# normallytangent/dune-eigensolver

Measured on AMD Instinct MI355X. Metric: Lanczos iters/sec + achieved SpMV HBM GB/s, 3D Poisson 256^3, higher is better.
Workload: dtype f64

## Files before the change

### dune-eigensolver_amd/csrc/drivers.cpp

```cpp
#include <algorithm>
#include <complex>
#include <cmath>
#include <cstdlib>
#include <cstring>
#include <numeric>
#include <string>
#include <vector>

#include "internal.h"

using namespace eigmi;

namespace {

bool distributed(const eig_mat_s &A) { return A.ctx->distributed(); }

struct PinnedDoubles {
  double *p = nullptr, *dev = nullptr;
  explicit PinnedDoubles(size_t n)
  {
    EIG_HIP(hipHostMalloc(reinterpret_cast<void **>(&p), (n ? n : 1) * sizeof(double), hipHostMallocMapped));
    EIG_HIP(hipHostGetDevicePointer(reinterpret_cast<void **>(&dev), p, 0));
  }
  ~PinnedDoubles()
// ... 1113 lines not shown
    EIG_CHECK(mode == EIG_ARNOLDI_STD || mode == EIG_ARNOLDI_GEN, EIG_ERR_ARG, "eig_arnoldi_shift_invert: bad mode");
    shift_invert_check(A, B);
    EIG_HIP(hipSetDevice(A->ctx->device));
    LuRef F;
    shift_invert_factor(A, B, lu, sigma, F);
    arnoldi_core(A, B, F, sigma, nev, ncv, tol, maxit, seed, mode == EIG_ARNOLDI_GEN, eval_re, eval_im, evec_host,
                 restarts);
  });
}

namespace {

struct LanczosBufs {
  DevBuf scal;
  DevBuf ictl;
  LanczosState st;
  double *carry;
  explicit LanczosBufs(int steps, int launches = 0)
      : scal((size_t)(4 * (steps + 2) + 6 * (launches + 2) + 8) * sizeof(double)),
        ictl((size_t)2 * (launches + 2) * sizeof(int))
  {
    double *b = scal.d();
    st.dsum = b;
    st.nsum = b + (steps + 2);
    st.alpha = b + 2 * (steps + 2);
    st.beta = b + 3 * (steps + 2);
    st.fred = b + 4 * (steps + 2);
    st.aux = st.fred + 3 * (launches + 2);
    carry = st.aux + 2 * (launches + 2);
    st.mu2 = carry + 4;
    st.pn = st.mu2 + 4;
    st.ctl = static_cast<int *>(ictl.p);
  }
};

enum { kPartOnly = 0, kPartFirst = 1, kPartSecond = 2 };
template <class Halo, class Launch>
void halo_split(eig_mat_s &A, hipEvent_t e0, hipEvent_t e1, Halo halo, Launch launch)
{
  eig_ctx_t ctx = A.ctx;
  hipStream_t s = ctx->stream;
  if (!distributed(A) || (A.recvs.empty() && A.sends.empty()))
  {
    launch(nullptr, 0, A.nslices, kPartOnly);
    return;
  }
  if (ctx->loop)
// ... 56 lines not shown
                        int nev, hipEvent_t halo_ev0, hipEvent_t halo_ev1, bool ev_external, int xch = 0)
{
  eig_ctx_t ctx = A.ctx;
  hipStream_t s = ctx->stream;
  auto mark = [&](int i) {
    if (ev && i < nev)
      EIG_HIP(hipEventRecordWithFlags(ev[i], s, ev_external ? hipEventRecordExternal : hipEventRecordDefault));
  };
  double *out = lb.st.fred + 3 * (i64)L;
  FusedLaunch fl{lb.st, L, force, xch & kXchPublish};
  FusedLaunch fl_first{lb.st, L, force, 0};
  mark(0);
  halo_split(
      A, halo_ev0, halo_ev1, [&](hipStream_t hs) { halo_exchange(A, P, hs, nullptr, 2); },
      [&](const i32 *sl, i64 first, i64 count, int part) {
        launch_lanczos_fused(A, P, Pout, part == kPartFirst ? fl_first : fl, sl, first, count,
                             part == kPartSecond ? lb.carry : nullptr, part == kPartFirst ? lb.carry : out, 0, s,
                             ctx->red);
      });
  mark(1);
  if (!(xch & kXchPublish)) allreduce_sum(ctx, out, 3, s);
  mark(2);
  mark(3);
  mark(4);
}

void init_start(eig_mat_s &A, double *U0, const double *u0, unsigned seed)
{
  eig_ctx_t ctx = A.ctx;
  hipStream_t s = ctx->stream;
  EIG_HIP(hipMemsetAsync(U0, 0, A.window * sizeof(double), s));
  const i64 n = A.nb_rows * A.br;
  if (u0)
// ... 13 lines not shown
}

struct eig_lanczos_s {
  eig_mat_s *A = nullptr;
  int max_steps = 0, k = 0;
  bool fused = false;
  bool pipe = false;
  hipEvent_t hp = nullptr, ha = nullptr;
  int L = 0, max_launches = 0;
  DevBuf *B[4] = {nullptr, nullptr, nullptr, nullptr};
  LanczosBufs *lb = nullptr;
  hipEvent_t h0 = nullptr, h1 = nullptr;
  hipGraph_t graph = nullptr;
  hipGraphExec_t gexec = nullptr;
  int g_steps = 0, g_flags = 0;
  std::vector<hipEvent_t> g_ev;
  void drop_graph()
  {
    if (gexec) (void)hipGraphExecDestroy(gexec);
    if (graph) (void)hipGraphDestroy(graph);
    for (auto &e : g_ev) (void)hipEventDestroy(e);
    gexec = nullptr;
    graph = nullptr;
    g_ev.clear();
    g_steps = 0;
  }
  ~eig_lanczos_s()
  {
    drop_graph();
    for (auto *b : B) delete b;
    delete lb;
    if (h0) (void)hipEventDestroy(h0);
    if (h1) (void)hipEventDestroy(h1);
    if (hp) (void)hipEventDestroy(hp);
    if (ha) (void)hipEventDestroy(ha);
  }
};

namespace {

// ... 200 lines not shown
        if (i) EIG_HIP(hipMemsetAsync(ws->B[i]->d(), 0, ws->B[i]->bytes(), s));
      }
      double *U0 = ws->pipe ? ws->B[0]->d() : ws->fused ? ws->B[2]->d() : ws->B[0]->d();
      init_start(*A, U0, u0, seed);
      ws->lb = new LanczosBufs(max_steps, ws->max_launches);
      launch_nrm2sq(A->nb_rows * A->br, U0 + A->own_offset, ws->lb->st.nsum, 0, s, ctx->red);
      if (ws->fused)
      {
        if (!ws->pipe)
        {
          EIG_HIP(hipMemsetAsync(ws->B[0]->d(), 0, 2 * wb, s));
          EIG_HIP(hipMemcpy2DAsync(ws->B[0]->d(), 2 * sizeof(double), U0, sizeof(double), sizeof(double),
                                   A->window, hipMemcpyDeviceToDevice, s));
        }
        EIG_HIP(hipMemsetAsync(ws->lb->st.ctl, 0, ws->lb->ictl.bytes(), s));
        const double mu2[2] = {A->diag_sum, (double)(A->nb_rows * A->br)};
        EIG_HIP(hipMemcpyAsync(ws->lb->st.mu2, mu2, sizeof(mu2), hipMemcpyHostToDevice, s));
        allreduce_sum(ctx, ws->lb->st.mu2, 2, s);
      }
      allreduce_sum(ctx, ws->lb->st.nsum, 1, s);
      EIG_HIP(hipEventCreateWithFlags(&ws->h0, hipEventDisableTiming));
      EIG_HIP(hipEventCreateWithFlags(&ws->h1, hipEventDisableTiming));
      EIG_HIP(hipEventCreateWithFlags(&ws->hp, hipEventDisableTiming));
      EIG_HIP(hipEventCreateWithFlags(&ws->ha, hipEventDisableTiming));
      EIG_HIP(hipStreamSynchronize(s));
    }
    catch (...)
    {
      delete ws;
      throw;
// ... 65 lines not shown
    EIG_CHECK(!ws->fused || ws->L + steps <= ws->max_launches, EIG_ERR_ARG, "fused Lanczos: launch capacity exhausted");
    ws->drop_graph();
    eig_ctx_t ctx = ws->A->ctx;
    EIG_HIP(hipSetDevice(ctx->device));
    ws->g_steps = steps;
    ws->g_flags = flags;
    ws->g_ev = make_events(steps, events_per_step(flags));
    if (captured) *captured = 0;
    if (ctx->loop) return;
    hipStream_t s = ctx->stream;
    march_prepare(*ws->A);
    EIG_HIP(hipStreamSynchronize(s));
    EIG_HIP(hipStreamBeginCapture(s, hipStreamCaptureModeRelaxed));
    hipGraph_t g = nullptr;
    bool ok = true;
    try
    {
      enqueue_steps(*ws, steps, events_per_step(flags), ws->g_ev.data(), true);
    }
    catch (...)
    {
      ok = false;
    }
    hipError_t e = hipStreamEndCapture(s, &g);
    if (!ok || e != hipSuccess || !g)
    {
      if (g) (void)hipGraphDestroy(g);
      (void)hipGetLastError();
      return;
    }
    ws->graph = g;
    if (hipGraphInstantiate(&ws->gexec, g, nullptr, nullptr, 0) != hipSuccess)
    {
      (void)hipGetLastError();
      (void)hipGraphDestroy(g);
      ws->graph = nullptr;
      ws->gexec = nullptr;
      return;
    }
    if (captured) *captured = 1;
  });
}

extern "C" int eig_lanczos_replay(eig_lanczos_t ws, eig_timing *timing)
{
  return guard(ws ? ws->A->ctx : nullptr, [&] {
    EIG_CHECK(ws && ws->g_steps > 0, EIG_ERR_ARG, "eig_lanczos_replay: nothing captured");
    eig_ctx_t ctx = ws->A->ctx;
    EIG_HIP(hipSetDevice(ctx->device));
    hipStream_t s = ctx->stream;
    const int steps = ws->g_steps;
    const int nps = events_per_step(ws->g_flags);
    const int target = ws->k + steps;
    if (ws->gexec)
      EIG_HIP(hipGraphLaunch(ws->gexec, s));
    else
      enqueue_steps(*ws, steps, nps, ws->g_ev.data(), false);
    EIG_HIP(hipStreamSynchronize(s));
    if (ws->fused) ws->L += steps;
    else ws->k += steps;
    read_timing(ws->g_ev, steps, nps, timing);
    ws->drop_graph();
    if (ws->fused) fused_settle(*ws, target, nps, timing);
  });
}

extern "C" int eig_lanczos_tridiag(eig_lanczos_t ws, int *k, double *alpha_host, double *beta_host)
{
  return guard(ws ? ws->A->ctx : nullptr, [&] {
    EIG_CHECK(ws, EIG_ERR_ARG, "eig_lanczos_tridiag: null workspace");
// ... 24 lines not shown
    EIG_HIP(hipStreamSynchronize(ctx->stream));
    check_step_exchange(*ws);
    if (k) *k = ws->k;
    if (alpha_host && ws->k > 0)
      EIG_HIP(hipMemcpy(alpha_host, ws->lb->st.alpha, ws->k * sizeof(double), hipMemcpyDeviceToHost));
    if (beta_host) EIG_HIP(hipMemcpy(beta_host, ws->lb->st.beta, (ws->k + 1) * sizeof(double), hipMemcpyDeviceToHost));
  });
}

extern "C" int eig_lanczos_info(eig_lanczos_t ws, int *steps, int *launches)
{
  return guard(ws ? ws->A->ctx : nullptr, [&] {
    EIG_CHECK(ws, EIG_ERR_ARG, "eig_lanczos_info: null workspace");
    if (steps) *steps = ws->k;
    if (launches) *launches = ws->fused ? ws->L : ws->k;
  });
}

extern "C" int eig_lanczos_destroy(eig_lanczos_t ws)
{
  if (!ws) return EIG_OK;
  (void)hipSetDevice(ws->A->ctx->device);
  (void)hipStreamSynchronize(ws->A->ctx->stream);
  delete ws;
  return EIG_OK;
}

extern "C" int eig_lanczos_run(eig_mat_t A, int steps, const double *u0, unsigned seed, int flags, double *alpha_host,
                               double *beta_host, eig_timing *timing)
{
// ... 110 lines not shown
```

### dune-eigensolver_amd/csrc/internal.h

```cpp
#pragma once
#include <hip/hip_runtime.h>
#include <rccl/rccl.h>

#include <complex>
#include <condition_variable>
#include <cstdint>
#include <mutex>
#include <new>
#include <stdexcept>
#include <string>
#include <memory>
#include <vector>

#include "../../include/eigmi.h"

namespace eigmi {

typedef int64_t i64;
typedef int32_t i32;
typedef uint64_t u64;

struct Error : std::runtime_error {
  int code;
  Error(int c, const std::string &m) : std::runtime_error(m), code(c) {}
// ... 223 lines not shown


void launch_spmv(const eig_mat_s &A, const double *x, double *y, const i32 *slices, i64 first, i64 count,
                 hipStream_t s, bool keep = false);

struct LanczosState {
  double *dsum;
  double *nsum;
  double *alpha;
  double *beta;
  double *fred;
  int *ctl;
  double *aux;
  double *mu2;
  double *pn;
};
enum { kFusedModeStep = 0, kFusedModePost = 1, kFusedModeHalt = 2 };
struct FusedLaunch {
  LanczosState st;
  int L;
  int force;
  int xch = 0;
};
enum { kXchPublish = 2 };
void launch_lanczos_fused(const eig_mat_s &A, const double *P, double *Pout, const FusedLaunch &fl,
                          const i32 *slices, i64 first, i64 count, const double *carry, double *out, int ticket,
                          hipStream_t s, ReduceWS red);
void launch_lanczos_pipe(const eig_mat_s &A, double *T, double *UZ, const double *S, const FusedLaunch &fl,
                         double *out, hipStream_t s, ReduceWS red);
void launch_fused_tail(const LanczosState &st, int L, hipStream_t s);
bool march_geometry(const eig_mat_s &A, i64 &D, int chunk = 64);
bool march_split_active(const eig_mat_s &A);
int march_variant(const eig_mat_s &A, bool fused);
extern const i32 kMarchInteriorTag;
bool box_prepare(const eig_mat_s &A);
inline bool box_spmm_applies(const eig_mat_s &A, i64 m)
{
  return m > 0 && m % 8 == 0 && box_prepare(A) && (A.box_ctab != nullptr || m % 32 == 0);
}
int box_cols(const eig_mat_s &A);
// ... 233 lines not shown
```

### dune-eigensolver_amd/csrc/k_spmv.hip

```cpp
#include "internal.h"
#include "march_variants.h"
#include "reduce_dev.h"
#include "xch_dev.h"

namespace eigmi {

constexpr int kWaves = kStreamThreads / 64;

template <int R>
struct Vec;
template <>
struct Vec<1> {
  typedef double d;
  typedef i32 i;
};
template <>
struct Vec<2> {
  typedef double d __attribute__((ext_vector_type(2)));
  typedef i32 i __attribute__((ext_vector_type(2)));
};
template <>
struct Vec<4> {
  typedef double d __attribute__((ext_vector_type(4)));
  typedef i32 i __attribute__((ext_vector_type(4)));
// ... 669 lines not shown

constexpr double kFusedTau = 1e-2;
enum { kFusedStep = 0, kFusedPost = 1, kFusedHalt = 2, kFusedRepair = 3, kFusedNoop = 4 };

struct FusedArgs {
  double *nsum, *alpha, *beta;
  const double *fred;
  int *ctl;
  double *aux;
  const double *mu2;
  double *pn;
  int L;
  int force;
  int xch;
  Mailbox mb;
};

struct FusedStep {
  int j, act;
  double c, nt, ap, bk, gam, sig, mu, rn, rm;
};

__device__ __forceinline__ FusedStep fused_begin(const FusedArgs &f)
{
  FusedStep s;
  const int cj = f.ctl[2 * f.L], mode = f.ctl[2 * f.L + 1];
  const double mu0 = f.mu2[0], mu1 = f.mu2[1];
  const int Lp = f.L > 0 ? f.L - 1 : 0;
  const double fd = f.fred[3 * Lp], fq = f.fred[3 * Lp + 1], fm = f.fred[3 * Lp + 2];
  const double ax0 = f.aux[2 * f.L], ax1 = f.aux[2 * f.L + 1], pnl = f.pn[f.L], ns0 = f.nsum[0];
  s.j = cj;
  s.mu = mu0 / mu1;
  s.c = s.ap = s.bk = s.gam = s.rn = s.rm = 0.0;
  s.nt = 1.0;
  const int j = s.j;
  if (mode == kFusedHalt) s.act = kFusedHalt;
  else if (f.force && (j == 0 || mode != kFusedStep)) s.act = kFusedNoop;
  else if (mode == kFusedPost)
  {
    const double mex = fm;
    s.rn = ax0;
    s.rm = ax1;
    s.nt = mex;
    if (!(mex > 0.0)) s.act = kFusedHalt;
    else
// ... 59 lines not shown
          f.beta[j] = 0.0;
        }
        nm = kFusedHalt;
        break;
      default:
        nm = mode;
        if (mode == kFusedPost)
        {
          f.aux[2 * f.L + 2] = f.aux[2 * f.L];
          f.aux[2 * f.L + 3] = f.aux[2 * f.L + 1];
        }
        break;
    }
    f.ctl[2 * f.L + 2] = nj;
    f.ctl[2 * f.L + 3] = nm;
    f.pn[f.L + 1] = (s.act == kFusedStep || s.act == kFusedPost) ? s.nt : pnl;
  }
  return s;
}

__device__ __forceinline__ void fused_idle(double *out)
{
  if (blockIdx.x == 0 && threadIdx.x < 3) out[threadIdx.x] = 0.0;
}

template <int U>
__device__ __forceinline__ void fused_finish(double (&v)[3], double *partials, unsigned *ticket, double *tot,
                                             double *out, const double *carry, const FusedArgs &fa)
{
  if (grid_sum<3, kStreamThreads, U>(v, partials, ticket, tot))
  {
    if (fa.xch & kXchPublish)
    {
      if (carry)
      {
        if (threadIdx.x < 3) tot[threadIdx.x] += carry[threadIdx.x];
        __syncthreads();
      }
      xch_exchange(fa.mb, tot);
      if (threadIdx.x < 3) out[threadIdx.x] = tot[threadIdx.x];
    }
    else if (threadIdx.x < 3)
      out[threadIdx.x] = carry ? (carry[threadIdx.x] + tot[threadIdx.x]) : tot[threadIdx.x];
  }
// ... 1170 lines not shown
  double d = 0.0, q2 = 0.0, m2 = 0.0;
  if constexpr (kTraits<UNI>.geo2_path())
  {
    FusedStep fs{};
    bool begun = false;
    auto epi = [&](int, int w, double acc, dpair pc) {
      const double uk = pc.x - fs.c * pc.y;
      double ti = (acc - fs.mu * uk) * fs.sig;
      if (fs.j > 0) ti = ti - fs.gam * pc.y;
      march_store(mp, dpair{ti, uk}, Pout + (unsigned)w);
      d += ti * uk;
      q2 += ti * ti;
      m2 += uk * uk;
    };
    auto pre = [&](XPair &x) {
      fs = fused_begin(fa);
      begun = true;
      x.c = fs.c;
      return fs.act == kFusedStep || fs.act == kFusedPost;
    };
    march_rows<MT, 2, SPAN1, UNI>(A, mp, own, lane, wave, XPair{P, 0.0}, epi, pre);
    if (!begun) fs = fused_begin(fa);
    if (fs.act == kFusedHalt || fs.act == kFusedNoop)
    {
      if (!(fa.xch & kXchPublish))
      {
        fused_idle(out);
        return;
      }
      d = q2 = m2 = 0.0;
    }
    if (fs.act == kFusedRepair)
    {
      const i64 r0 = mp.zb * mp.D, r1 = std::min<i64>(nrows, (mp.zb + mp.nplanes) * mp.D);
      m2 = fused_repair_rows(r0, r1, own, fs.c, P, Pout);
    }
    double v[3] = {d, q2, m2};
// ... 30 lines not shown
      }
    };
    march_rows<MT, 2, SPAN1, UNI>(A, mp, own, lane, wave, XPair{P, c}, epi);
  }
  double v[3] = {d, q2, m2};
  fused_finish<8>(v, partials, ticket, tot, out, nullptr, fa);
}

__global__ __launch_bounds__(kStreamThreads) void k_lanczos_pipe(i64 n, double *__restrict__ T,
                                                                 dpair *__restrict__ UZ,
                                                                 const double *__restrict__ S, FusedArgs fa,
                                                                 double *__restrict__ out, double *partials,
                                                                 unsigned *ticket)
{
  __shared__ double tot[3];
  const FusedStep fs = fused_begin(fa);
  if (fs.act == kFusedHalt || fs.act == kFusedNoop)
  {
    fused_idle(out);
    return;
  }
  const double c = fs.c, gam = fs.gam, sig = fs.sig, mu = fs.mu;
  const bool k0 = fs.j > 0;
  const i64 stride = (i64)gridDim.x * kStreamThreads;
  double d = 0.0, q2 = 0.0, m2 = 0.0;
  if (fs.act == kFusedRepair)
  {
    for (i64 i = (i64)blockIdx.x * kStreamThreads + threadIdx.x; i < n; i += stride)
    {
      const double u = T[i] - c * UZ[i].x;
      T[i] = u;
// ... 301 lines not shown
        const double di = __builtin_nontemporal_load(dinv + r);
        const dpair bb = __builtin_nontemporal_load(Bb + (unsigned)w * 4u);
        const dpair xo = __builtin_nontemporal_load(Yb + (unsigned)w * 4u);
        const double gd = gamma * di;
        const double o0 = omega * (pcur.x + gd * (bb.x - acc.x) - xo.x) + xo.x;
        const double o1 = omega * (pcur.y + gd * (bb.y - acc.y) - xo.y) + xo.y;
        __builtin_nontemporal_store(dpair{o0, o1}, Yb + (unsigned)w * 4u);
      }
    }
    pm = pcur;
    pcur = pP;
    amP = aP;
  }
}

__global__ void k_fused_tail(double *nsum, double *beta, const double *fred, const int *ctl, const double *aux, int L)
{
  if (threadIdx.x != 0 || blockIdx.x != 0) return;
  const int j = ctl[2 * L], mode = ctl[2 * L + 1];
  if (mode == kFusedPost)
  {
    const double mex = fred[3 * (L - 1) + 2];
    nsum[j] = mex;
    beta[j] = mex > 0.0 ? sqrt(mex) * aux[2 * L] / aux[2 * L + 1] : 0.0;
  }
  else if (j == 0)
    beta[0] = sqrt(nsum[0]);
}

template <class K>
static int grid_for_slices(K kernel, i64 count, int num_cu)
{
  static thread_local std::pair<const void *, int> cache{nullptr, 0};
  int per_cu = 0;
  if (cache.first == (const void *)kernel) per_cu = cache.second;
  else
  {
// ... 380 lines not shown
  {                                                                                                          \
    const int m_ = image_mode(A);                                                                            \
    if (m_ == kExplicit) EIG_LZ(R_, kExplicit);                                                              \
    else if (m_ == kStencil) EIG_LZ(R_, kStencil);                                                           \
    else if (m_ == kSym8) EIG_LZ(R_, kSym8);                                                                 \
    else if (m_ == kSym32) EIG_LZ(R_, kSym32);                                                               \
    else if (m_ == kSymN8) EIG_LZ(R_, kSymN8);                                                               \
    else if (m_ == kSymN32) EIG_LZ(R_, kSymN32);                                                               \
    else EIG_LZ(R_, kMixed);                                                                                 \
  }
  EIG_LZM(1)
#undef EIG_LZM
#undef EIG_LZ
}

void launch_lanczos_fused(const eig_mat_s &A, const double *P, double *Pout, const FusedLaunch &fl,
                          const i32 *slices, i64 first, i64 count, const double *carry, double *out, int ticket,
                          hipStream_t s, ReduceWS red)
{
  EIG_CHECK(lanczos_blocks_ok(A), EIG_ERR_BLOCKSIZE, "Lanczos step: square blocks 1..4 only (blocks: one rank)");
  FusedArgs fa{fl.st.nsum, fl.st.alpha, fl.st.beta, fl.st.fred, fl.st.ctl, fl.st.aux, fl.st.mu2, fl.st.pn, fl.L,
               fl.force, 0, Mailbox{}};
  if (fl.xch)
  {
    EIG_CHECK(A.ctx->step_exchange(), EIG_ERR_ARG, "fused step: in-kernel exchange without the mailbox");
    fa.xch = fl.xch & kXchPublish;
    fa.mb = A.ctx->mbox->dev;
  }
#define EIG_LFB(B_)                                                                                          \
  if (A.br == B_)                                                                                            \
  {                                                                                                          \
    hipLaunchKernelGGL((k_lanczos_fused_blk<B_>),                                                            \
                       dim3(grid_for_slices(k_lanczos_fused_blk<B_>, count, A.ctx->num_cu)),                 \
                       dim3(kStreamThreads), 0, s, A.nb_rows, A.slice_ptr, slices, first, count, A.val, A.col, \
                       reinterpret_cast<const dpair *>(P), reinterpret_cast<dpair *>(Pout), fa, out, carry,   \
                       red.partials, red.ticket(ticket));                                                    \
    return;                                                                                                  \
  }
  EIG_LFB(2) EIG_LFB(3) EIG_LFB(4)
#undef EIG_LFB
  if (!carry)
  {
    const int mode = image_mode(A);
    MarchPlan mp = launch_plan(A, mode, slices, first, count, true);
    if (mp.nseg > 0)
    {
      if (march_down_variant(mp.uni) && ((A.tune_cache & 24) == 24 || (kMarch2lSerpentine && !(A.tune_cache & 24))))
        mp.down = fl.L & 1;
      march_launch(MarchDispatch{}, A, mode, mp.uni, [&](auto mt, auto span1, auto uni) {
        hipLaunchKernelGGL((k_lanczos_fused_march<decltype(mt), span1(), uni()>), dim3(march_grid(mp)),
                           dim3(kStreamThreads), 0, s, A.nb_rows, A.own_offset, sell_b1(A), mp,
                           reinterpret_cast<const dpair *>(P), reinterpret_cast<dpair *>(Pout), fa, out, red.partials,
                           red.ticket(ticket));
      });
      return;
    }
  }
#define EIG_LF_(R_, M_, CPF_)                                                                                 \
  hipLaunchKernelGGL((k_lanczos_fused_b1<R_, M_, CPF_>),                                                     \
                     dim3(grid_for_slices(k_lanczos_fused_b1<R_, M_, CPF_>, count, A.ctx->num_cu)),           \
                     dim3(kStreamThreads), 0, s, A.nb_rows, A.own_offset, sell_b1(A), slices, first, count,      \
                     reinterpret_cast<const dpair *>(P), reinterpret_cast<dpair *>(Pout), fa, out, carry,        \
                     red.partials, red.ticket(ticket))
#define EIG_LF(R_, M_)                                                                                        \
  do                                                                                                          \
  {                                                                                                           \
    if (sell_cpf(A, true) && (M_ == kExplicit || M_ == kMixed)) EIG_LF_(R_, M_, true);                        \
    else EIG_LF_(R_, M_, false);                                                                              \
  } while (0)
#define EIG_LFM(R_)                                                                                           \
  {                                                                                                           \
    const int m_ = image_mode(A);                                                                             \
    if (m_ == kExplicit) EIG_LF(R_, kExplicit);                                                               \
    else if (m_ == kStencil) EIG_LF(R_, kStencil);                                                            \
    else if (m_ == kSym8) EIG_LF(R_, kSym8);                                                                  \
    else if (m_ == kSym32) EIG_LF(R_, kSym32);                                                                \
    else if (m_ == kSymN8) EIG_LF(R_, kSymN8);                                                                \
    else if (m_ == kSymN32) EIG_LF(R_, kSymN32);                                                              \
    else EIG_LF(R_, kMixed);                                                                                  \
  }
  EIG_LFM(1)
#undef EIG_LFM
#undef EIG_LF
#undef EIG_LF_
}

void launch_lanczos_pipe(const eig_mat_s &A, double *T, double *UZ, const double *S, const FusedLaunch &fl,
                         double *out, hipStream_t s, ReduceWS red)
{
  EIG_CHECK(A.br == 1 && A.bc == 1, EIG_ERR_BLOCKSIZE, "Lanczos driver: 1x1 blocks only");
  const i64 n = A.nb_rows, own = A.own_offset;
  EIG_CHECK((own & 1) == 0 && (((uintptr_t)T | (uintptr_t)UZ | (uintptr_t)S) & 15) == 0, EIG_ERR_ARG,
            "pipelined Lanczos: vectors must be 16-B aligned");
  const FusedArgs fa{fl.st.nsum, fl.st.alpha, fl.st.beta, fl.st.fred, fl.st.ctl, fl.st.aux, fl.st.mu2, fl.st.pn, fl.L,
                     fl.force, 0, Mailbox{}};
  const i64 per = 2LL * kStreamThreads;
  const int G = (int)std::max<i64>(1, std::min<i64>(kStreamBlocks, (n + per - 1) / per));
  hipLaunchKernelGGL(k_lanczos_pipe, dim3(G), dim3(kStreamThreads), 0, s, n, T + own,
                     reinterpret_cast<dpair *>(UZ) + own, S + own, fa, out, red.partials, red.ticket(0));
}

void launch_fused_tail(const LanczosState &st, int L, hipStream_t s)
{
  hipLaunchKernelGGL(k_fused_tail, dim3(1), dim3(64), 0, s, st.nsum, st.beta, st.fred, st.ctl, st.aux, L);
}

static bool gspans(const eig_mat_s &A, i64 &P, GSpans &sp)
{
  if (!A.sym_val || A.sym_nd < 3) return false;
  const int nd = A.sym_nd;
  auto kof = [&](i64 d) {
    for (int k = 0; k < nd; ++k)
      if (A.sym_off[k] == d) return k;
    return -1;
  };
  if (kof(1) < 0 || kof(-1) < 0) return false;
  const auto [klo, khi] = far_spans(A);
  for (int kp = nd - 1; kp >= khi; --kp)
  {
// ... 197 lines not shown
```

### dune-eigensolver_amd/csrc/reduce_dev.h

```cpp
#pragma once
#include <hip/hip_runtime.h>

namespace eigmi {

__device__ __forceinline__ double wave_sum(double v)
{
#pragma unroll
  for (int off = 32; off > 0; off >>= 1) v += __shfl_down(v, off, 64);
  return v;
}

__device__ __forceinline__ void st_sc1(double *p, double v)
{
  __hip_atomic_store(reinterpret_cast<unsigned long long *>(p), __double_as_longlong(v), __ATOMIC_RELAXED,
                     __HIP_MEMORY_SCOPE_AGENT);
}
__device__ __forceinline__ double ld_sc1(const double *p)
{
  unsigned long long b = __hip_atomic_load(reinterpret_cast<const unsigned long long *>(p), __ATOMIC_RELAXED,
                                           __HIP_MEMORY_SCOPE_AGENT);
  return __longlong_as_double((long long)b);
}

__device__ __forceinline__ bool ticket_arrive(unsigned *t, unsigned bid, unsigned nblk)
// ... 83 lines not shown
#pragma unroll
      for (int i = 0; i < NV; ++i) acc[i] += vals[u][i];
  }
  double r[NV];
  block_sum<NV, NT>(acc, r);
  if (threadIdx.x == 0)
  {
#pragma unroll
    for (int i = 0; i < NV; ++i) tot[i] = r[i];
    ticket_reset(ticket);
  }
  __syncthreads();
  return true;
}

template <int NT>
__device__ bool grid_sum2(const double *vals, int E, double *part, double *spart, unsigned *t, unsigned bid,
                          unsigned nblk, double *out)
{
  __shared__ unsigned s_flag;
  for (int e = threadIdx.x; e < E; e += NT) st_sc1(&part[(size_t)bid * E + e], vals[e]);
  asm volatile("s_waitcnt vmcnt(0)" ::: "memory");
  __syncthreads();
  constexpr unsigned L = 32;
  const unsigned shard = bid & 7u;
  const unsigned shard_n = nblk / 8u + ((shard < nblk % 8u) ? 1u : 0u);
  const unsigned nshards = nblk < 8u ? nblk : 8u;
  if (threadIdx.x == 0)
    s_flag = __hip_atomic_fetch_add(t + shard * L, 1u, __ATOMIC_RELAXED, __HIP_MEMORY_SCOPE_AGENT) == shard_n - 1u;
  __syncthreads();
// ... 106 lines not shown
```

### dune-eigensolver_amd/eigmi.py

```python
import atexit
import ctypes
import itertools
import os
import weakref

import numpy as np

_HERE = os.path.dirname(os.path.abspath(__file__))
LIB_PATH = os.path.join(_HERE, "lib", "libeigmi_san.so" if os.environ.get("EIGMI_LIB_VARIANT") == "san"
                        else "libeigmi.so")

EIG_OK, EIG_ERR_SHAPE, EIG_ERR_BLOCKSIZE, EIG_ERR_HIP, EIG_ERR_RCCL, EIG_ERR_BREAKDOWN, EIG_ERR_ARG, EIG_ERR_NODEVICE = range(8)
ORTHO_MGS, ORTHO_CHOLQR, ORTHO_CHOLQR_SPLIT = 0, 1, 2
ORTHO_GRID = 0x100
ORTHO_NO_COOP = 0x200
ORTHO_ONE_WG = 0x400


def ORTHO_LOOKAHEAD(L):
    return int(L) << 12

MAT_NO_BAND, MAT_BAND_GATHER, MAT_NO_STENCIL, MAT_NO_MARCH, MAT_NO_CLASS, MAT_NO_UNIFORM = 1, 2, 4, 8, 16, 32
TRSV_AUTO, TRSV_BLOCKINV, TRSV_STAGED, TRSV_CSR = 0, 1, 2, 3
TRSV_KINDS = {None: TRSV_AUTO, "auto": TRSV_AUTO, "blockinv": TRSV_BLOCKINV, "staged": TRSV_STAGED, "csr": TRSV_CSR}
# ... 127 lines not shown
    "eig_orthonormalize_mv8": (_int, [_vp, _i64, _i64, _vp, _int]),
    "eig_orthonormalize_passes": (_int, [_vp, ctypes.POINTER(ctypes.c_int)]),
    "eig_orthonormalize_naive": (_int, [_vp, _i64, _i64, _vp]),
    "eig_b_orthonormalize_mv8": (_int, [_vp, _i64, _vp, _vp]),
    "eig_random_mv8": (_int, [_vp, _i64, _i64, _u, _vp]),
    "eig_random_normal": (_int, [_i64, _u, _vp]),
    "eig_standard_largest": (_int, [_vp, _dbl, _dbl, _int, _int, _u, _vp, _vp, ctypes.POINTER(_int), _int]),
    "eig_lanczos_run": (_int, [_vp, _int, _vp, _u, _int, _vp, _vp, ctypes.POINTER(Timing)]),
    "eig_lanczos_solve": (_int, [_vp, _int, _int, _int, _u, _vp, _vp, _vp]),
    "eig_lanczos_create": (_int, [_vp, _int, _vp, _u, ctypes.POINTER(_vp)]),
    "eig_lanczos_create_ex": (_int, [_vp, _int, _vp, _u, _int, ctypes.POINTER(_vp)]),
    "eig_lanczos_step": (_int, [_vp, _int, _int, ctypes.POINTER(Timing)]),
    "eig_lanczos_tridiag": (_int, [_vp, ctypes.POINTER(_int), _vp, _vp]),
    "eig_lanczos_destroy": (_int, [_vp]),
    "eig_lanczos_info": (_int, [_vp, ctypes.POINTER(_int), ctypes.POINTER(_int)]),
    "eig_lanczos_capture": (_int, [_vp, _int, _int, ctypes.POINTER(_int)]),
    "eig_lanczos_ws_info": (_int, [_vp, ctypes.POINTER(_int), ctypes.c_char_p, _int, ctypes.POINTER(_i64)]),
    "eig_lanczos_replay": (_int, [_vp, ctypes.POINTER(Timing)]),
    "eig_lu_create": (_int, [_vp, _i64, _vp, _vp, _vp, _vp, _vp, _vp, _vp, _vp, _vp, _int, ctypes.POINTER(_vp)]),
    "eig_lu_create_bcsr": (_int, [_vp, _i64, _int, _vp, _vp, _vp, ctypes.POINTER(_vp)]),
    "eig_lu_info": (_int, [_vp, ctypes.POINTER(_i64), ctypes.POINTER(_i64), ctypes.POINTER(_i64), ctypes.POINTER(_int)]),
    "eig_lu_export": (_int, [_vp, _vp, _vp, _vp, _vp, _vp, _vp, _vp, _vp, _vp]),
    "eig_lu_destroy": (_int, [_vp]),
    "eig_inverse_mv8": (_int, [_vp, _i64, _vp, _vp]),
    "eig_standard_inverse": (_int, [_vp, _vp, _dbl, _dbl, _int, _int, _u, _vp, _vp, ctypes.POINTER(_int), _int]),
    "eig_generalized_inverse": (_int, [_vp, _vp, _vp, _dbl, _dbl, _dbl, _int, _int, _u, _vp, _vp, ctypes.POINTER(_int),
                                       _int]),
    "eig_shift_invert_solve": (_int, [_vp, _vp, _vp, _dbl, _int, _int, _dbl, _int, _u, _vp, _vp, ctypes.POINTER(_int)]),
    "eig_shift_invert_solve_ex": (_int, [_vp, _vp, _vp, _dbl, _int, _int, _dbl, _int, _u, _vp, _vp,
                                         ctypes.POINTER(_int), _int]),
# ... 481 lines not shown
        c = _int(0)
        self.A.ctx.check(lib.eig_lanczos_capture(self.h, steps, _tflags(timed),
                                                 ctypes.byref(c)))
        return bool(c.value)

    def replay(self):
        t = Timing()
        self.A.ctx.check(lib.eig_lanczos_replay(self.h, ctypes.byref(t)))
        return t

    def info(self):
        k, L = _int(0), _int(0)
        self.A.ctx.check(lib.eig_lanczos_info(self.h, ctypes.byref(k), ctypes.byref(L)))
        return k.value, L.value

    def tridiag(self):
        k = _int(0)
        self.A.ctx.check(lib.eig_lanczos_tridiag(self.h, ctypes.byref(k), None, None))
        alpha = np.zeros(max(k.value, 1))
        beta = np.zeros(k.value + 1)
        self.A.ctx.check(lib.eig_lanczos_tridiag(self.h, ctypes.byref(k), _np_ptr(alpha), _np_ptr(beta)))
        return alpha[:k.value], beta

    def close(self):
        if self.h and self.A.h and self.A.ctx.h:
            lib.eig_lanczos_destroy(self.h)
        self.h = None

    def __del__(self):
        try:
# ... 403 lines not shown
```

### include/eigmi.h

```cpp
#ifndef EIGMI_H
#define EIGMI_H

#include <stddef.h>
#include <stdint.h>

#ifdef __cplusplus
extern "C" {
#endif

#define EIGMI_VERSION_MAJOR 0
#define EIGMI_VERSION_MINOR 1

enum eig_status {
  EIG_OK = 0,
  EIG_ERR_SHAPE = 1,
  EIG_ERR_BLOCKSIZE = 2,
  EIG_ERR_HIP = 3,
  EIG_ERR_RCCL = 4,
  EIG_ERR_BREAKDOWN = 5,
  EIG_ERR_ARG = 6,
  EIG_ERR_NODEVICE = 7
};

typedef struct eig_ctx_s *eig_ctx_t;
// ... 148 lines not shown
  EIG_LANCZOS_FUSED = 4,
  EIG_LANCZOS_PIPELINED = 8,
  EIG_LANCZOS_AUTO = 16
};
int eig_lanczos_run(eig_mat_t A, int steps, const double *u0, unsigned seed, int flags,
                    double *alpha_host, double *beta_host, eig_timing *timing);

typedef struct eig_lanczos_s *eig_lanczos_t;
int eig_lanczos_create(eig_mat_t A, int max_steps, const double *u0, unsigned seed, eig_lanczos_t *ws);
int eig_lanczos_create_ex(eig_mat_t A, int max_steps, const double *u0, unsigned seed, int flags,
                          eig_lanczos_t *ws);
int eig_lanczos_step(eig_lanczos_t ws, int steps, int flags, eig_timing *timing);
int eig_lanczos_tridiag(eig_lanczos_t ws, int *k, double *alpha_host, double *beta_host);
int eig_lanczos_destroy(eig_lanczos_t ws);
int eig_lanczos_info(eig_lanczos_t ws, int *steps, int *launches);
int eig_lanczos_ws_info(eig_lanczos_t ws, int *variant, char *name, int name_len, int64_t *bytes);
int eig_lanczos_capture(eig_lanczos_t ws, int steps, int flags, int *captured);
int eig_lanczos_replay(eig_lanczos_t ws, eig_timing *timing);

enum eig_which { EIG_WHICH_LA = 0, EIG_WHICH_SA = 1 };
int eig_lanczos_solve(eig_mat_t A, int nev, int ncv, int which, unsigned seed, double *eval_host,
                      double *evec_host, double *resid_host);

typedef struct eig_lu_s *eig_lu_t;
int eig_lu_create(eig_ctx_t ctx, int64_t n, const int64_t *Lp, const int64_t *Lj, const double *Lx,
                  const int64_t *Up, const int64_t *Ui, const double *Ux, const int64_t *P, const int64_t *Q,
                  const double *Rs, int do_recip, eig_lu_t *lu);
int eig_lu_create_bcsr(eig_ctx_t ctx, int64_t nb_rows, int br, const int64_t *rowptr, const int32_t *col,
                       const double *vals, eig_lu_t *lu);
int eig_lu_info(eig_lu_t lu, int64_t *n, int64_t *lnz, int64_t *unz, int *do_recip);
// ... 89 lines not shown
```

Before: 5459.

## Defer fused Lanczos grid reduction to the next launch's prologue

When the fused Lanczos step runs on one device with a small enough grid, each block now writes its per-block partial sums into a double-buffered part array instead of doing a ticketed grid-wide reduction with a last-block finish. The next launch, or the tail kernel, reads the block count and sums up to 512 partials at its start to rebuild the dot products. This removes the atomic ticket and the last-block serialization at the end of each step. In exchange every block in the following kernel does a small extra load and block reduction, and a deferred-launch counter plus API is added for inspection.

After: 5443. About the same (-0.3%).

```diff
diff --git a/dune-eigensolver_amd/csrc/drivers.cpp b/dune-eigensolver_amd/csrc/drivers.cpp
--- a/dune-eigensolver_amd/csrc/drivers.cpp
+++ b/dune-eigensolver_amd/csrc/drivers.cpp
@@ -1151,11 +1151,14 @@
 struct LanczosBufs {
   DevBuf scal;
   DevBuf ictl;
+  DevBuf part;
   LanczosState st;
   double *carry;
+  long long deferred = 0;
   explicit LanczosBufs(int steps, int launches = 0)
       : scal((size_t)(4 * (steps + 2) + 6 * (launches + 2) + 8) * sizeof(double)),
-        ictl((size_t)2 * (launches + 2) * sizeof(int))
+        ictl((size_t)2 * (launches + 2) * sizeof(int)),
+        part(launches ? (size_t)2 * kFusedPartStride * sizeof(double) : 0)
   {
     double *b = scal.d();
     st.dsum = b;
@@ -1168,6 +1171,7 @@
     st.mu2 = carry + 4;
     st.pn = st.mu2 + 4;
     st.ctl = static_cast<int *>(ictl.p);
+    st.part = part.d();
   }
 };
 
@@ -1254,9 +1258,9 @@
   halo_split(
       A, halo_ev0, halo_ev1, [&](hipStream_t hs) { halo_exchange(A, P, hs, nullptr, 2); },
       [&](const i32 *sl, i64 first, i64 count, int part) {
-        launch_lanczos_fused(A, P, Pout, part == kPartFirst ? fl_first : fl, sl, first, count,
-                             part == kPartSecond ? lb.carry : nullptr, part == kPartFirst ? lb.carry : out, 0, s,
-                             ctx->red);
+        lb.deferred += launch_lanczos_fused(A, P, Pout, part == kPartFirst ? fl_first : fl, sl, first, count,
+                                            part == kPartSecond ? lb.carry : nullptr,
+                                            part == kPartFirst ? lb.carry : out, 0, s, ctx->red);
       });
   mark(1);
   if (!(xch & kXchPublish)) allreduce_sum(ctx, out, 3, s);
@@ -1300,6 +1304,7 @@
   hipGraph_t graph = nullptr;
   hipGraphExec_t gexec = nullptr;
   int g_steps = 0, g_flags = 0;
+  long long g_deferred = 0;
   std::vector<hipEvent_t> g_ev;
   void drop_graph()
   {
@@ -1310,6 +1315,7 @@
     graph = nullptr;
     g_ev.clear();
     g_steps = 0;
+    g_deferred = 0;
   }
   ~eig_lanczos_s()
   {
@@ -1540,6 +1546,7 @@
                                    A->window, hipMemcpyDeviceToDevice, s));
         }
         EIG_HIP(hipMemsetAsync(ws->lb->st.ctl, 0, ws->lb->ictl.bytes(), s));
+        EIG_HIP(hipMemsetAsync(ws->lb->st.part, 0, ws->lb->part.bytes(), s));
         const double mu2[2] = {A->diag_sum, (double)(A->nb_rows * A->br)};
         EIG_HIP(hipMemcpyAsync(ws->lb->st.mu2, mu2, sizeof(mu2), hipMemcpyHostToDevice, s));
         allreduce_sum(ctx, ws->lb->st.mu2, 2, s);
@@ -1635,6 +1642,7 @@
     EIG_HIP(hipStreamBeginCapture(s, hipStreamCaptureModeRelaxed));
     hipGraph_t g = nullptr;
     bool ok = true;
+    const long long deferred0 = ws->lb->deferred;
     try
     {
       enqueue_steps(*ws, steps, events_per_step(flags), ws->g_ev.data(), true);
@@ -1643,6 +1651,8 @@
     {
       ok = false;
     }
+    const long long g_deferred = ws->lb->deferred - deferred0;
+    ws->lb->deferred = deferred0;
     hipError_t e = hipStreamEndCapture(s, &g);
     if (!ok || e != hipSuccess || !g)
     {
@@ -1659,6 +1669,7 @@
       ws->gexec = nullptr;
       return;
     }
+    ws->g_deferred = g_deferred;
     if (captured) *captured = 1;
   });
 }
@@ -1674,7 +1685,10 @@
     const int nps = events_per_step(ws->g_flags);
     const int target = ws->k + steps;
     if (ws->gexec)
+    {
       EIG_HIP(hipGraphLaunch(ws->gexec, s));
+      ws->lb->deferred += ws->g_deferred;
+    }
     else
       enqueue_steps(*ws, steps, nps, ws->g_ev.data(), false);
     EIG_HIP(hipStreamSynchronize(s));
@@ -1729,6 +1743,14 @@
     EIG_CHECK(ws, EIG_ERR_ARG, "eig_lanczos_info: null workspace");
     if (steps) *steps = ws->k;
     if (launches) *launches = ws->fused ? ws->L : ws->k;
+  });
+}
+
+extern "C" int eig_lanczos_deferred(eig_lanczos_t ws, int64_t *launches)
+{
+  return guard(ws ? ws->A->ctx : nullptr, [&] {
+    EIG_CHECK(ws && launches, EIG_ERR_ARG, "eig_lanczos_deferred: bad argument");
+    *launches = ws->lb->deferred;
   });
 }
 
diff --git a/dune-eigensolver_amd/csrc/internal.h b/dune-eigensolver_amd/csrc/internal.h
--- a/dune-eigensolver_amd/csrc/internal.h
+++ b/dune-eigensolver_amd/csrc/internal.h
@@ -261,7 +261,10 @@
   double *aux;
   double *mu2;
   double *pn;
-};
+  double *part;
+};
+constexpr int kFusedDeferCap = 512;
+constexpr int kFusedPartStride = 2 + 3 * kFusedDeferCap;
 enum { kFusedModeStep = 0, kFusedModePost = 1, kFusedModeHalt = 2 };
 struct FusedLaunch {
   LanczosState st;
@@ -270,7 +273,7 @@
   int xch = 0;
 };
 enum { kXchPublish = 2 };
-void launch_lanczos_fused(const eig_mat_s &A, const double *P, double *Pout, const FusedLaunch &fl,
+bool launch_lanczos_fused(const eig_mat_s &A, const double *P, double *Pout, const FusedLaunch &fl,
                           const i32 *slices, i64 first, i64 count, const double *carry, double *out, int ticket,
                           hipStream_t s, ReduceWS red);
 void launch_lanczos_pipe(const eig_mat_s &A, double *T, double *UZ, const double *S, const FusedLaunch &fl,
diff --git a/dune-eigensolver_amd/csrc/k_spmv.hip b/dune-eigensolver_amd/csrc/k_spmv.hip
--- a/dune-eigensolver_amd/csrc/k_spmv.hip
+++ b/dune-eigensolver_amd/csrc/k_spmv.hip
@@ -707,21 +707,63 @@
   int force;
   int xch;
   Mailbox mb;
+  double *part;
+  int defer;
 };
+
+static_assert(kFusedPartStride == 2 + 3 * (int)kDeferSlots && kFusedDeferCap == (int)kDeferSlots, "internal.h / reduce_dev.h");
+__device__ __forceinline__ double *fused_part(const FusedArgs &f, int L) { return f.part + (L & 1) * kFusedPartStride; }
+
+__device__ __forceinline__ void fused_part_load(const FusedArgs &f, double (&p)[2][3])
+{
+  deferred_load<3>(fused_part(f, f.L + 1) + 2, p);
+}
+
+struct FusedIn {
+  int cj, mode;
+  unsigned dcount;
+  double mu0, mu1, fd, fq, fm, ax0, ax1, pnl, ns0;
+};
+__device__ __forceinline__ FusedIn fused_in(const FusedArgs &f, bool defer = true)
+{
+  FusedIn in;
+  in.cj = f.ctl[2 * f.L];
+  in.mode = f.ctl[2 * f.L + 1];
+  in.mu0 = f.mu2[0];
+  in.mu1 = f.mu2[1];
+  const int Lp = f.L > 0 ? f.L - 1 : 0;
+  in.fd = f.fred[3 * Lp];
+  in.fq = f.fred[3 * Lp + 1];
+  in.fm = f.fred[3 * Lp + 2];
+  in.ax0 = f.aux[2 * f.L];
+  in.ax1 = f.aux[2 * f.L + 1];
+  in.pnl = f.pn[f.L];
+  in.ns0 = f.nsum[0];
+  in.dcount = 0;
+  if (defer && f.L > 0)
+    in.dcount = (unsigned)__builtin_amdgcn_readfirstlane(*reinterpret_cast<const int *>(fused_part(f, f.L + 1)));
+  return in;
+}
 
 struct FusedStep {
   int j, act;
   double c, nt, ap, bk, gam, sig, mu, rn, rm;
 };
 
-__device__ __forceinline__ FusedStep fused_begin(const FusedArgs &f)
+__device__ __forceinline__ FusedStep fused_begin_sums(const FusedArgs &f, const FusedIn &in, const double (&tot)[3])
 {
   FusedStep s;
-  const int cj = f.ctl[2 * f.L], mode = f.ctl[2 * f.L + 1];
-  const double mu0 = f.mu2[0], mu1 = f.mu2[1];
+  const int cj = in.cj, mode = in.mode;
+  const unsigned dcount = in.dcount;
+  const double mu0 = in.mu0, mu1 = in.mu1, ax0 = in.ax0, ax1 = in.ax1, pnl = in.pnl, ns0 = in.ns0;
   const int Lp = f.L > 0 ? f.L - 1 : 0;
-  const double fd = f.fred[3 * Lp], fq = f.fred[3 * Lp + 1], fm = f.fred[3 * Lp + 2];
-  const double ax0 = f.aux[2 * f.L], ax1 = f.aux[2 * f.L + 1], pnl = f.pn[f.L], ns0 = f.nsum[0];
+  double fd = in.fd, fq = in.fq, fm = in.fm;
+  if (dcount)
+  {
+    fd = tot[0];
+    fq = tot[1];
+    fm = tot[2];
+  }
   s.j = cj;
   s.mu = mu0 / mu1;
   s.c = s.ap = s.bk = s.gam = s.rn = s.rm = 0.0;
@@ -811,9 +853,33 @@
     }
     f.ctl[2 * f.L + 2] = nj;
     f.ctl[2 * f.L + 3] = nm;
+    *reinterpret_cast<int *>(fused_part(f, f.L)) =
+        (f.defer && s.act != kFusedHalt && s.act != kFusedNoop) ? (int)gridDim.x : 0;
+    if (dcount)
+    {
+      double *fr = const_cast<double *>(f.fred) + 3 * Lp;
+      fr[0] = fd;
+      fr[1] = fq;
+      fr[2] = fm;
+    }
     f.pn[f.L + 1] = (s.act == kFusedStep || s.act == kFusedPost) ? s.nt : pnl;
   }
   return s;
+}
+
+enum { kDeferNever = 0, kDeferRare = 1, kDeferEager = 2 };
+template <int MODE = kDeferRare>
+__device__ __forceinline__ FusedStep fused_begin(const FusedArgs &f)
+{
+  double tot[3] = {0.0, 0.0, 0.0};
+  const FusedIn in = fused_in(f, MODE != kDeferNever);
+  if (MODE == kDeferEager || in.dcount)
+  {
+    double p[2][3];
+    fused_part_load(f, p);
+    deferred_sum<3>(p, in.dcount, tot);
+  }
+  return fused_begin_sums(f, in, tot);
 }
 
 __device__ __forceinline__ void fused_idle(double *out)
@@ -825,6 +891,17 @@
 __device__ __forceinline__ void fused_finish(double (&v)[3], double *partials, unsigned *ticket, double *tot,
                                              double *out, const double *carry, const FusedArgs &fa)
 {
+  if (!ticket)
+  {
+    double bs[3];
+    block_sum<3, kStreamThreads>(v, bs);
+    if (threadIdx.x == 0)
+    {
+#pragma unroll
+      for (int i = 0; i < 3; ++i) partials[blockIdx.x * 3 + i] = bs[i];
+    }
+    return;
+  }
   if (grid_sum<3, kStreamThreads, U>(v, partials, ticket, tot))
   {
     if (fa.xch & kXchPublish)
@@ -2025,13 +2102,13 @@
       m2 += uk * uk;
     };
     auto pre = [&](XPair &x) {
-      fs = fused_begin(fa);
+      fs = fused_begin<kDeferEager>(fa);
       begun = true;
       x.c = fs.c;
       return fs.act == kFusedStep || fs.act == kFusedPost;
     };
     march_rows<MT, 2, SPAN1, UNI>(A, mp, own, lane, wave, XPair{P, 0.0}, epi, pre);
-    if (!begun) fs = fused_begin(fa);
+    if (!begun) fs = fused_begin<kDeferEager>(fa);
     if (fs.act == kFusedHalt || fs.act == kFusedNoop)
     {
       if (!(fa.xch & kXchPublish))
@@ -2092,7 +2169,7 @@
                                                                  unsigned *ticket)
 {
   __shared__ double tot[3];
-  const FusedStep fs = fused_begin(fa);
+  const FusedStep fs = fused_begin<kDeferNever>(fa);
   if (fs.act == kFusedHalt || fs.act == kFusedNoop)
   {
     fused_idle(out);
@@ -2424,13 +2501,25 @@
   }
 }
 
-__global__ void k_fused_tail(double *nsum, double *beta, const double *fred, const int *ctl, const double *aux, int L)
-{
-  if (threadIdx.x != 0 || blockIdx.x != 0) return;
+__global__ void k_fused_tail(double *nsum, double *beta, double *fred, const int *ctl, const double *aux,
+                             const double *part, int L)
+{
+  part += ((L + 1) & 1) * kFusedPartStride;
+  const unsigned dcount = L > 0 ? (unsigned)__builtin_amdgcn_readfirstlane(*reinterpret_cast<const int *>(part)) : 0u;
+  double tot[3] = {0.0, 0.0, 0.0};
+  if (dcount)
+  {
+    double p[2][3];
+    deferred_load<3>(part + 2, p);
+    deferred_sum<3>(p, dcount, tot);
+  }
+  if (threadIdx.x != 0) return;
+  if (dcount)
+    for (int i = 0; i < 3; ++i) fred[3 * (L - 1) + i] = tot[i];
   const int j = ctl[2 * L], mode = ctl[2 * L + 1];
   if (mode == kFusedPost)
   {
-    const double mex = fred[3 * (L - 1) + 2];
+    const double mex = dcount ? tot[2] : fred[3 * (L - 1) + 2];
     nsum[j] = mex;
     beta[j] = mex > 0.0 ? sqrt(mex) * aux[2 * L] / aux[2 * L + 1] : 0.0;
   }
@@ -2841,13 +2930,26 @@
 #undef EIG_LZ
 }
 
-void launch_lanczos_fused(const eig_mat_s &A, const double *P, double *Pout, const FusedLaunch &fl,
+bool launch_lanczos_fused(const eig_mat_s &A, const double *P, double *Pout, const FusedLaunch &fl,
                           const i32 *slices, i64 first, i64 count, const double *carry, double *out, int ticket,
                           hipStream_t s, ReduceWS red)
 {
   EIG_CHECK(lanczos_blocks_ok(A), EIG_ERR_BLOCKSIZE, "Lanczos step: square blocks 1..4 only (blocks: one rank)");
   FusedArgs fa{fl.st.nsum, fl.st.alpha, fl.st.beta, fl.st.fred, fl.st.ctl, fl.st.aux, fl.st.mu2, fl.st.pn, fl.L,
-               fl.force, 0, Mailbox{}};
+               fl.force, 0, Mailbox{}, fl.st.part, 0};
+  const bool may_defer = !A.ctx->collectives() && !fl.xch && !carry && !fl.force && !(A.tune_cache & 32) &&
+                         out == fl.st.fred + 3 * (i64)fl.L;
+  double *partials = red.partials;
+  unsigned *tick = red.ticket(ticket);
+  auto grid_of = [&](i64 g) {
+    fa.defer = may_defer && g <= kFusedDeferCap;
+    if (fa.defer)
+    {
+      partials = fl.st.part + (fl.L & 1) * kFusedPartStride + 2;
+      tick = nullptr;
+    }
+    return dim3((unsigned)g);
+  };
   if (fl.xch)
   {
     EIG_CHECK(A.ctx->step_exchange(), EIG_ERR_ARG, "fused step: in-kernel exchange without the mailbox");
@@ -2857,12 +2959,12 @@
 #define EIG_LFB(B_)                                                                                          \
   if (A.br == B_)                                                                                            \
   {                                                                                                          \
-    hipLaunchKernelGGL((k_lanczos_fused_blk<B_>),                                                            \
-                       dim3(grid_for_slices(k_lanczos_fused_blk<B_>, count, A.ctx->num_cu)),                 \
+    const dim3 g_ = grid_of(grid_for_slices(k_lanczos_fused_blk<B_>, count, A.ctx->num_cu));                 \
+    hipLaunchKernelGGL((k_lanczos_fused_blk<B_>), g_,                                                        \
                        dim3(kStreamThreads), 0, s, A.nb_rows, A.slice_ptr, slices, first, count, A.val, A.col, \
                        reinterpret_cast<const dpair *>(P), reinterpret_cast<dpair *>(Pout), fa, out, carry,   \
-                       red.partials, red.ticket(ticket));                                                    \
-    return;                                                                                                  \
+                       partials, tick);                                                                      \
+    return fa.defer != 0;                                                                                    \
   }
   EIG_LFB(2) EIG_LFB(3) EIG_LFB(4)
 #undef EIG_LFB
@@ -2874,21 +2976,24 @@
     {
       if (march_down_variant(mp.uni) && ((A.tune_cache & 24) == 24 || (kMarch2lSerpentine && !(A.tune_cache & 24))))
         mp.down = fl.L & 1;
+      const dim3 grid = grid_of(march_grid(mp));
       march_launch(MarchDispatch{}, A, mode, mp.uni, [&](auto mt, auto span1, auto uni) {
-        hipLaunchKernelGGL((k_lanczos_fused_march<decltype(mt), span1(), uni()>), dim3(march_grid(mp)),
+        hipLaunchKernelGGL((k_lanczos_fused_march<decltype(mt), span1(), uni()>), grid,
                            dim3(kStreamThreads), 0, s, A.nb_rows, A.own_offset, sell_b1(A), mp,
-                           reinterpret_cast<const dpair *>(P), reinterpret_cast<dpair *>(Pout), fa, out, red.partials,
-                           red.ticket(ticket));
+                           reinterpret_cast<const dpair *>(P), reinterpret_cast<dpair *>(Pout), fa, out, partials,
+                           tick);
       });
-      return;
+      return fa.defer != 0;
     }
   }
 #define EIG_LF_(R_, M_, CPF_)                                                                                 \
-  hipLaunchKernelGGL((k_lanczos_fused_b1<R_, M_, CPF_>),                                                     \
-                     dim3(grid_for_slices(k_lanczos_fused_b1<R_, M_, CPF_>, count, A.ctx->num_cu)),           \
-                     dim3(kStreamThreads), 0, s, A.nb_rows, A.own_offset, sell_b1(A), slices, first, count,      \
-                     reinterpret_cast<const dpair *>(P), reinterpret_cast<dpair *>(Pout), fa, out, carry,        \
-                     red.partials, red.ticket(ticket))
+  do                                                                                                          \
+  {                                                                                                           \
+    const dim3 g_ = grid_of(grid_for_slices(k_lanczos_fused_b1<R_, M_, CPF_>, count, A.ctx->num_cu));         \
+    hipLaunchKernelGGL((k_lanczos_fused_b1<R_, M_, CPF_>), g_, dim3(kStreamThreads), 0, s, A.nb_rows,         \
+                       A.own_offset, sell_b1(A), slices, first, count, reinterpret_cast<const dpair *>(P),    \
+                       reinterpret_cast<dpair *>(Pout), fa, out, carry, partials, tick);                      \
+  } while (0)
 #define EIG_LF(R_, M_)                                                                                        \
   do                                                                                                          \
   {                                                                                                           \
@@ -2910,6 +3015,7 @@
 #undef EIG_LFM
 #undef EIG_LF
 #undef EIG_LF_
+  return fa.defer != 0;
 }
 
 void launch_lanczos_pipe(const eig_mat_s &A, double *T, double *UZ, const double *S, const FusedLaunch &fl,
@@ -2920,7 +3026,7 @@
   EIG_CHECK((own & 1) == 0 && (((uintptr_t)T | (uintptr_t)UZ | (uintptr_t)S) & 15) == 0, EIG_ERR_ARG,
             "pipelined Lanczos: vectors must be 16-B aligned");
   const FusedArgs fa{fl.st.nsum, fl.st.alpha, fl.st.beta, fl.st.fred, fl.st.ctl, fl.st.aux, fl.st.mu2, fl.st.pn, fl.L,
-                     fl.force, 0, Mailbox{}};
+                     fl.force, 0, Mailbox{}, fl.st.part, 0};
   const i64 per = 2LL * kStreamThreads;
   const int G = (int)std::max<i64>(1, std::min<i64>(kStreamBlocks, (n + per - 1) / per));
   hipLaunchKernelGGL(k_lanczos_pipe, dim3(G), dim3(kStreamThreads), 0, s, n, T + own,
@@ -2929,7 +3035,8 @@
 
 void launch_fused_tail(const LanczosState &st, int L, hipStream_t s)
 {
-  hipLaunchKernelGGL(k_fused_tail, dim3(1), dim3(64), 0, s, st.nsum, st.beta, st.fred, st.ctl, st.aux, L);
+  hipLaunchKernelGGL(k_fused_tail, dim3(1), dim3(kStreamThreads), 0, s, st.nsum, st.beta, st.fred, st.ctl, st.aux, st.part,
+                     L);
 }
 
 static bool gspans(const eig_mat_s &A, i64 &P, GSpans &sp)
diff --git a/dune-eigensolver_amd/csrc/reduce_dev.h b/dune-eigensolver_amd/csrc/reduce_dev.h
--- a/dune-eigensolver_amd/csrc/reduce_dev.h
+++ b/dune-eigensolver_amd/csrc/reduce_dev.h
@@ -121,6 +121,50 @@
   return true;
 }
 
+constexpr unsigned kDeferSlots = 512;
+
+template <int NV>
+__device__ __forceinline__ void deferred_load(const double *part, double (&p)[2][NV])
+{
+#pragma unroll
+  for (int h = 0; h < 2; ++h)
+#pragma unroll
+    for (int i = 0; i < NV; ++i) p[h][i] = part[(threadIdx.x + 256u * h) * NV + i];
+}
+
+__device__ __forceinline__ double lane0(double v)
+{
+  const long long b = __double_as_longlong(v);
+  const unsigned lo = (unsigned)__builtin_amdgcn_readfirstlane((int)b);
+  const unsigned hi = (unsigned)__builtin_amdgcn_readfirstlane((int)(b >> 32));
+  return __longlong_as_double((long long)(((unsigned long long)hi << 32) | lo));
+}
+
+template <int NV>
+__device__ __forceinline__ void deferred_sum(const double (&p)[2][NV], unsigned count, double (&tot)[NV])
+{
+  __shared__ double sh[4][NV];
+  const unsigned t = threadIdx.x;
+#pragma unroll
+  for (int i = 0; i < NV; ++i)
+  {
+    double a = 0.0;
+    a += t < count ? p[0][i] : 0.0;
+    a += t + 256u < count ? p[1][i] : 0.0;
+    const double r = wave_sum(a);
+    if ((t & 63u) == 0) sh[t >> 6][i] = r;
+  }
+  __syncthreads();
+#pragma unroll
+  for (int i = 0; i < NV; ++i)
+  {
+    double s = 0.0;
+#pragma unroll
+    for (int w = 0; w < 4; ++w) s += sh[w][i];
+    tot[i] = lane0(s);
+  }
+}
+
 template <int NT>
 __device__ bool grid_sum2(const double *vals, int E, double *part, double *spart, unsigned *t, unsigned bid,
                           unsigned nblk, double *out)
diff --git a/dune-eigensolver_amd/eigmi.py b/dune-eigensolver_amd/eigmi.py
--- a/dune-eigensolver_amd/eigmi.py
+++ b/dune-eigensolver_amd/eigmi.py
@@ -165,6 +165,7 @@
     "eig_lanczos_tridiag": (_int, [_vp, ctypes.POINTER(_int), _vp, _vp]),
     "eig_lanczos_destroy": (_int, [_vp]),
     "eig_lanczos_info": (_int, [_vp, ctypes.POINTER(_int), ctypes.POINTER(_int)]),
+    "eig_lanczos_deferred": (_int, [_vp, ctypes.POINTER(_i64)]),
     "eig_lanczos_capture": (_int, [_vp, _int, _int, ctypes.POINTER(_int)]),
     "eig_lanczos_ws_info": (_int, [_vp, ctypes.POINTER(_int), ctypes.c_char_p, _int, ctypes.POINTER(_i64)]),
     "eig_lanczos_replay": (_int, [_vp, ctypes.POINTER(Timing)]),
@@ -676,6 +677,11 @@
         self.A.ctx.check(lib.eig_lanczos_info(self.h, ctypes.byref(k), ctypes.byref(L)))
         return k.value, L.value
 
+    def deferred(self):
+        d = _i64(0)
+        self.A.ctx.check(lib.eig_lanczos_deferred(self.h, ctypes.byref(d)))
+        return d.value
+
     def tridiag(self):
         k = _int(0)
         self.A.ctx.check(lib.eig_lanczos_tridiag(self.h, ctypes.byref(k), None, None))
diff --git a/include/eigmi.h b/include/eigmi.h
--- a/include/eigmi.h
+++ b/include/eigmi.h
@@ -186,6 +186,7 @@
 int eig_lanczos_tridiag(eig_lanczos_t ws, int *k, double *alpha_host, double *beta_host);
 int eig_lanczos_destroy(eig_lanczos_t ws);
 int eig_lanczos_info(eig_lanczos_t ws, int *steps, int *launches);
+int eig_lanczos_deferred(eig_lanczos_t ws, int64_t *launches);
 int eig_lanczos_ws_info(eig_lanczos_t ws, int *variant, char *name, int name_len, int64_t *bytes);
 int eig_lanczos_capture(eig_lanczos_t ws, int steps, int flags, int *captured);
 int eig_lanczos_replay(eig_lanczos_t ws, eig_timing *timing);
```
